# Sleepwalking/libllsm2

Hardware: AMD Instinct MI355X
Metric: frames/sec (layer0 analyze+synth, 44.1 kHz, 5 ms hop) (higher is better)
Workload: dtype f32; 1 GPU; 1024 synthetic 1 s utterances per GPU, F0 120 Hz fixed, 44.1 kHz, 5 ms hop, layer0 analyze+synth, default options, f0_refine=0; utterances_per_gpu=1024, frames_per_utterance=200, parallelism=dp1

## Files before the change

### libllsm2_amd/csrc/engine.cpp

```cpp
#include <hip/hip_runtime.h>
#include <sched.h>

#include <algorithm>
#include <atomic>
#include <cctype>
#include <cmath>
#include <cstdio>
#include <cstring>
#include <map>
#include <mutex>
#include <string>
#include <vector>

#include "cheby.h"
#include "engine.h"
#include "kernels.h"
#include "llsm_gpu.h"
#include "plan.h"
#include "batch.h"

namespace lp = llsm_plan;

namespace {
struct HostConventions { int hann_periodic = 0, mavg_half = 3, filtfilt_pad = 15, interp1u_excl = 0, kalman_init = 0, lobe_1e6 = 133979, lf_rd_clamp = 0; } g_hconv;
// ... 1136 lines not shown
      int C = (int)((Ftot + NF_UNIT_DIV - 1) / NF_UNIT_DIV);
      C = std::max(4, (C + 1) & ~1);
      if(const char* e = std::getenv("LLSM_GPU_NOISE_UNIT")) C = std::max(2, std::atoi(e) & ~1);
      std::vector<int4> units;
      for(int u = 0; u < b -> lay.n_utt; u ++) {
        const int nf = b -> nfrm[u], nu = (nf + C - 1) / C;
        const int sz = nu > 0 ? (((nf + nu - 1) / nu) + 1) & ~1 : 2;
        for(int i0 = 0; i0 < nf; i0 += sz) units.push_back(make_int4(u, i0, std::min(i0 + sz, nf), 0));
      }
      b -> n_nf_units = (int)units.size();
      const double hop = (double)thop * fs;
      b -> nf_halo = (int)std::floor((b -> nfft_filt + 1) / std::max(hop, 1.0));
      if(upload_vec(b -> nf_units, units)) return -1;
    }
    std::vector<float> wf = make_hann(b -> nwin_filt);
    double s = 0; for(float v : wf) s += (double)v * v;
    b -> inv_wsqr = (float)(1.0 / s);
    if(upload_vec(b -> win_filt, wf)) return -1;
    b -> syn_fs = fs; b -> njobs_syn = 0;
  }
  if(so -> use_l1 && llsm_l1_prefetch_rows(b, so)) return -1;
  const size_t tplsz = (size_t)L.n_utt * nch * L.ntemplate_ext;
  if(b -> colored.alloc(tplsz) || b -> mid.alloc(tplsz) ||
     b -> iir_tmp.alloc((size_t)L.n_utt * nch * (L.ntemplate_ext + 32)) ||
     b -> env_cplx.alloc(F * nch * std::max(L.maxnhar_e, 1)) || b -> yexc.alloc(Y)) return -1;
  float* white = (float*)b -> arr[LLSM_GPU_WHITE];
  {
    const void* key[3] = {b -> colored.p, b -> mid.p, b -> iir_tmp.p};
    if(b -> njobs_syn == 0 || std::memcmp(key, b -> key_syn, sizeof(key))) {
      if(build_jobs(b, 1, fs, nullptr, white)) return -1;
      std::memcpy(b -> key_syn, key, sizeof(key));
    }
  }
  BatchDev d = batch_dev(b, fs);
  LaunchCtx* P = & c -> lc;
  float* ysin = (float*)b -> arr[LLSM_GPU_YSIN];
  if(! use_injected_white) RUN(launch_white(P, d, white, L.ntemplate_ext, b -> d_ny.p, seed));
  RUN(launch_filtfilt(P, b -> jobs_syn.p, b -> njobs_syn, b -> sections.p));
  RUN(launch_env_params(P, d, b -> env_cplx.p));
  RUN(launch_excite_env(P, d, b -> colored.p, L.ntemplate_ext, b -> env_hits.p, b -> env_cplx.p,
    b -> nwin_env, b -> win_env.p, b -> nch_active, b -> d_y_off.p, b -> d_ny.p, b -> max_ny, fs,
    b -> yexc.p));
  float* ynoise = (float*)b -> arr[LLSM_GPU_YNOISE];
  static const bool fused_ok = [] { const char* e = std::getenv("LLSM_GPU_NOISE_OLA"); return !(e && e[0] == '0'); }();
  int fused = -2;
  if(fused_ok)
    fused = launch_noise_filter_ola(P, d, b -> nf_units.p, b -> n_nf_units, b -> nf_halo, b -> yexc.p,
      b -> d_y_off.p, b -> d_ny.p, b -> fnyq, fs, b -> nwin_filt, b -> win_filt.p, hann_sym(b -> nwin_filt), b -> inv_wsqr,
      ilog2(b -> nfft_filt), ynoise);
  if(fused != 0 && fused != -2) {
    llsm_set_error(std::string("launch_noise_filter_ola failed: ") + hipGetErrorString((hipError_t)fused));
    return -1;
  }
  float* yout = (float*)b -> arr[LLSM_GPU_Y];
  if(so -> use_l1) {
    if(fused == -2) {
      if(b -> nframes.alloc(F * b -> nfft_filt) || b -> live.alloc(F)) return -1;
      if(b -> nfft_filt > LLSM_LDS_FFT_MAX &&
         llsm_engine_big_fft(c, b -> nfft_filt, (size_t)llsm_big_fft_grid((size_t)b -> nfft_filt + b -> nfft_filt / 2 + 1) * (size_t)(b -> nfft_filt + b -> nfft_filt / 2 + 1))) return -1;
      HIP_OK(hipMemsetAsync(ysin, 0, Y * sizeof(float), c -> stream));
      RUN(launch_noise_filter(P, d, b -> yexc.p, b -> d_y_off.p, b -> d_ny.p, b -> fnyq, fs,
        b -> nwin_filt, b -> win_filt.p, b -> inv_wsqr, b -> nfft_filt, ilog2(b -> nfft_filt),
        c -> tw, c -> tw_nmax, b -> nframes.p, b -> live.p, 0));
      RUN(launch_ola_noise_mix(P, d, b -> nframes.p, b -> live.p, b -> nfft_filt,
        b -> d_y_off.p, b -> d_ny.p, b -> max_ny, fs, ysin, ynoise, yout));
    }
    return llsm_l1_synthesize_harmonics(b, so, ynoise, ysin, yout);
  }
  RUN(launch_synth_ola(P, d, b -> sin_units.p, b -> n_sin_units, b -> sin_halo, b -> nwin_sin, b -> win_sin.p,
    std::min(L.maxnhar, 2048), b -> d_y_off.p, b -> d_ny.p, fused == 0 ? ynoise : nullptr, ysin, 1,
    fused == 0 ? yout : nullptr));
  if(fused == -2) {
// ... 88 lines not shown
```

### libllsm2_amd/csrc/kernels.h

```cpp
#ifndef LLSM_AMD_KERNELS_H
#define LLSM_AMD_KERNELS_H

#include <hip/hip_runtime.h>
#include <stddef.h>
#include "cheby.h"
#include "packed.h"

struct FiltSectionD {
  double b[5];
  double a[5];
  double zi[4];
  double M[6][16];
  double H[IIR_SEG][4];
};

#ifndef KAL_CHUNK
#define KAL_CHUNK 8
#endif
struct FiltJob {
  const float* src;
  float* dst;
  float* mid;
  float* tmp;
  int n;
// ... 66 lines not shown
int launch_psd_frames(LaunchCtx* P, const BatchDev& d, const float* xres, int nwin,
  const float* win, float inv_wpow, int N, int logN, const float2* tw, int tw_nmax,
  float* psd_log);
int launch_kalman(LaunchCtx* P, const BatchDev& d, const float* env, const float* psd_log,
  float* ck, int nspec);
int launch_white(LaunchCtx* P, const BatchDev& d, float* white, int ntemplate_ext,
  const int* out_len, unsigned long long seed);
int launch_env_frames(LaunchCtx* P, const BatchDev& d, float fs_syn, int nwin,
  const float* win, float* envf);
#define LLSM_EXC_HITS 3
int launch_env_params(LaunchCtx* P, const BatchDev& d, float2* cplx);
int launch_pack_frames(LaunchCtx* P, const BatchDev& d, const LlsmPackedLayout& L, float* out, float* const* dst_tab);
int launch_unpack_frames(LaunchCtx* P, const BatchDev& d, const LlsmPackedLayout& L, const float* in, const float* const* src_tab);
int launch_scatter_outputs(LaunchCtx* P, int n_utt, int max_ny, const float* y, const float* ysin, const float* ynoise,
  const int* y_off, const int* ny, float* const* tab);
int launch_env_plan(LaunchCtx* P, int max_ny, int max_nfrm, int nwin_env, float thop, float fs, int2* hits, int* over);
int launch_excite_env(LaunchCtx* P, const BatchDev& d, const float* colored, int ntemplate_ext,
  const int2* hits, const float2* cplx, int nwin_env, const float* win, int nch_active,
  const int* out_off, const int* out_len, int max_len, float fs_syn, float* yexc);
int launch_noise_filter(LaunchCtx* P, const BatchDev& d, const float* yexc,
  const int* out_off, const int* out_len, float fnyq_conf, float fs_syn, int nwin,
  const float* win, float inv_wsqr, int N, int logN, const float2* tw, int tw_nmax,
  float* nframes_out, int* live, int rt);
int launch_noise_filter_ola(LaunchCtx* P, const BatchDev& d, const int4* units, int nunits, int halo,
  const float* yexc, const int* out_off, const int* out_len, float fnyq_conf, float fs_syn, int nwin,
  const float* win, int wsym, float inv_wsqr, int logN, float* ynoise);
int launch_ola_noise_mix(LaunchCtx* P, const BatchDev& d, const float* nframes_in,
  const int* live, int N, const int* out_off, const int* out_len,
  int max_len, float fs_syn, const float* ysin, float* ynoise, float* y);

int launch_utt_fftsize(LaunchCtx* P, const BatchDev& d, int nmax, int* nfft_u);
int launch_harm_pp(LaunchCtx* P, const BatchDev& d, const float* sig, size_t sig_stride, int nsig,
  const int* nfft_u, int maxnhar, float norm_base, const float2* tw, int tw_nmax, int lds_n,
  int* nhar_out, float* ampl, float* phse);
int launch_rt_template(LaunchCtx* P, const float* colored, int ntemplate_ext, int nch, int nch_active,
  int ntemplate, int S, float* tpl);
int launch_rt_rings(LaunchCtx* P, int S, float* mod, float* sinr, float* noiser, int cap, int nch,
  int mod_curr, int sin_curr, int noise_curr, int nhop, int nwin, const float* envf,
  const float* frames_sin, const float* f0, const int* has_nm, const int* nhar);
int launch_rt_rings_excite(LaunchCtx* P, int S, float* mod, float* sinr, float* noiser, int cap, int nch,
  int mod_curr, int sin_curr, int noise_curr, int nhop, int nwin, const float* envf, const float* frames_sin,
  const float* f0, const int* has_nm, const int* nhar, const float* tpl, float* excr, int ntemplate, int exc_curr,
  int exc_cycle, float* exc_frame);
int launch_rt_excite(LaunchCtx* P, int S, const float* mod, const float* tpl, float* excr, int cap,
  int nch, int ntemplate, int mod_curr, int exc_curr, int exc_cycle, int curr_nhop, int nx,
  int nwin_frame, float* exc_frame);
int launch_rt_mix(LaunchCtx* P, int S, float* noiser, const float* sinr, int cap, int noise_curr,
  int sin_curr, int sin_pos, int nfft, const float* nframes_in, const int* live, int next_nhop,
  int out_stride, float* out);
// ... 88 lines not shown
```

### libllsm2_amd/csrc/kernels.hip

```cpp
#include <hip/hip_runtime.h>
#include <stdint.h>
#include <climits>
#include <algorithm>
#include <cstdlib>
#include <cstring>
#include <map>
#include <mutex>
#include <utility>

#include "kernels.h"
#include "plan.h"

namespace lp = llsm_plan;

#pragma clang fp contract(fast)

#include "dev_common.h"
#include "synth_frame.h"
#include "launch.h"
#if defined(LLSM_KBENCH_EXPERIMENTS)
#include "../../tools/kbench_experiments.h"
#else
#if defined(IIR_FAKE_L2) || defined(IIR_GEN_EXPERIMENT) || defined(RT2_TIMING) || defined(HT_TABLE_EXPERIMENT) || defined(KAL_BREAK)
#error "timing-experiment switches need -DLLSM_KBENCH_EXPERIMENTS (tools/kbench.py); the product library is never built with them"
// ... 1983 lines not shown
__global__ __launch_bounds__(256) void k_env_params(
  const float* __restrict__ f0, const int* __restrict__ nhar_e,
  const float* __restrict__ eamp, const float* __restrict__ ephs, int nframes, int nch, int me,
  float2* __restrict__ cplx) {
  const size_t tid = (size_t)blockIdx.x * 256 + threadIdx.x;
  if(tid >= (size_t)nframes * nch * me) return;
  const int g = (int)(tid / ((size_t)nch * me)), k = (int)(tid % me);
  const int K = f0[g] > 0 ? min(nhar_e[g], me) : 0;
  float2 v = make_float2(0.0f, 0.0f);
  if(k < K) {
    float sn, co; sincosf(ephs[tid], & sn, & co);
    const float a = eamp[tid];
    v = make_float2(a * co, a * sn);
  }
  cplx[tid] = v;
}

#define EXC_HITS 3
#ifndef EXC_FAST
#define EXC_FAST 1
#endif
#define EXC_SLOTS 8
template <int NCH, int ME>
__global__ __launch_bounds__(256) void k_excite_env(
  const float* __restrict__ colored, int ntemplate_ext, const int2* __restrict__ hits,
  const float2* __restrict__ cplx, const float* __restrict__ edc, const float* __restrict__ f0,
  int nwin_env, const float* __restrict__ win, int nch, int me, int nch_active,
  const int* __restrict__ frm_off, const int* __restrict__ nfrm,
  const int* __restrict__ out_off, const int* __restrict__ out_len, float thop, float fs,
  float* __restrict__ yexc) {
  __shared__ float2 s_cp[EXC_SLOTS][NCH * ME];
  __shared__ float s_off[EXC_SLOTS][NCH];
  __shared__ float s_turn[EXC_SLOTS];
  const int u = blockIdx.y;
  const int b0 = blockIdx.x * 256, idx = b0 + threadIdx.x;
  const int ny = out_len[u];
  if(b0 >= ny) return;
  const int nf = nfrm[u], fo = frm_off[u];
  const float hop = lp::fmul(thop, fs);
  const int imin = max(0, (int)((float)b0 / hop) - 1);
  for(int t = threadIdx.x; t < EXC_SLOTS * NCH * ME; t += 256) {
    const int sl = t / (NCH * ME), r = t % (NCH * ME), c = r / ME, k = r % ME;
    const int i = imin + sl;
    float2 v = make_float2(0.0f, 0.0f);
    if(i < nf && c < nch && k < me) v = cplx[((size_t)(fo + i) * nch + c) * me + k];
    s_cp[sl][r] = v;
// ... 1 lines not shown
  if(threadIdx.x < EXC_SLOTS * NCH) {
    const int sl = threadIdx.x / NCH, c = threadIdx.x % NCH, i = imin + sl;
    s_off[sl][c] = (i < nf && c < nch) ? edc[(size_t)(fo + i) * nch + c] : 0.0f;
  }
  if(threadIdx.x < EXC_SLOTS) {
    const int i = imin + threadIdx.x;
    s_turn[threadIdx.x] = i < nf ? f0[fo + i] / fs : 0.0f;
  }
  __syncthreads();
  if(idx >= ny) return;
  const int ntemplate = min(20000, ny);
  int b; float r;
  const int a = lp::stretch_index(idx, ntemplate, ny, 128, & b, & r);
  const int half = nwin_env / 2;
  float e[NCH];
#pragma unroll
  for(int c = 0; c < NCH; c ++) e[c] = 0.0f;
#pragma unroll
  for(int hh = 0; hh < EXC_HITS; hh ++) {
    const int2 hit = hits[(size_t)idx * EXC_HITS + hh];
    if(hit.x < 0 || hit.x >= nf) continue;
    const int sl = hit.x - imin, j = hit.y;
    const float w = win[j];
    if(sl >= 0 && sl < EXC_SLOTS) {
      const float tn = s_turn[sl];
      float z1r = 1.0f, z1i = 0.0f;
#if EXC_FAST
      if(tn > 0) { const float ph = tn * (float)(j - half); z1r = __builtin_amdgcn_cosf(ph); z1i = __builtin_amdgcn_sinf(ph); }
#else
      if(tn > 0) cs_turns((double)tn * (double)(j - half), & z1r, & z1i);
#endif
      float zr[ME], zi[ME];
      zr[0] = z1r; zi[0] = z1i;
#pragma unroll
      for(int k = 1; k < ME; k ++) {
        zr[k] = zr[k - 1] * z1r - zi[k - 1] * z1i; zi[k] = zr[k - 1] * z1i + zi[k - 1] * z1r;
      }
#pragma unroll
      for(int c = 0; c < NCH; c ++) {
        float y = 0.0f;
#pragma unroll
        for(int k = 0; k < ME; k ++) {
          const float2 av = s_cp[sl][c * ME + k];
          y += av.x * zr[k] - av.y * zi[k];
        }
        e[c] += fmaxf(y + s_off[sl][c], 1e-8f) * w;
      }
    } else {
      const int g = fo + hit.x;
      const float f = f0[g];
      float z1r = 1.0f, z1i = 0.0f;
      if(f > 0) cs_turns((double)(f / fs) * (double)(j - half), & z1r, & z1i);
      for(int c = 0; c < nch; c ++) {
        float y = 0.0f, zr = z1r, zi = z1i;
        for(int k = 0; k < me; k ++) {
          const float2 av = cplx[((size_t)g * nch + c) * me + k];
          y += av.x * zr - av.y * zi;
          const float nr = zr * z1r - zi * z1i, ni = zr * z1i + zi * z1r;
          zr = nr; zi = ni;
        }
        const float val = fmaxf(y + edc[(size_t)g * nch + c], 1e-8f) * w;
#pragma unroll
        for(int cc = 0; cc < NCH; cc ++) if(cc == c) e[cc] += val;
      }
    }
  }
  const float xf = b >= 0 ? __frsqrt_rn(2.0f * r * (r - 1.0f) + 1.0f) : 1.0f;
  float acc = 0;
#pragma unroll
  for(int c = 0; c < NCH; c ++) {
    if(c < nch_active) {
      const float* tpl = colored + ((size_t)u * nch + c) * ntemplate_ext;
      float v = tpl[a];
      if(b >= 0) {
        v *= 1.0f - r;
        v += tpl[b] * r;
        v *= xf;
      }
#if EXC_FAST
      v *= __builtin_amdgcn_sqrtf(e[c]);
#else
      v *= sqrtf(e[c]);
#endif
      acc += v;
    }
  }
  yexc[(size_t)out_off[u] + idx] = acc;
}


#ifndef EXC4_WPE
#define EXC4_WPE 4
#endif
#define EXC4_SLOTS 16
template <int NCH, int ME>
__global__ __launch_bounds__(256, EXC4_WPE) void k_excite_env4(
  const float* __restrict__ colored, int ntemplate_ext, const int2* __restrict__ hits,
  const float2* __restrict__ cplx, const float* __restrict__ edc, const float* __restrict__ f0,
  int nwin_env, const float* __restrict__ win, int nch, int me, int nch_active,
  const int* __restrict__ frm_off, const int* __restrict__ nfrm,
  const int* __restrict__ out_off, const int* __restrict__ out_len, float thop, float fs,
  float* __restrict__ yexc) {
  __shared__ __attribute__((aligned(16))) float2 s_cp[EXC4_SLOTS][NCH * ME];
  __shared__ float s_off[EXC4_SLOTS][NCH];
  __shared__ float s_turn[EXC4_SLOTS];
  __shared__ float2 s_w[EXC4_SLOTS];
  const int u = blockIdx.y;
  const int ny = out_len[u];
  const int nt = min(20000, ny);
  const bool tiled = ny > nt;
// ... 515 lines not shown
      const int lo = max(0, k - mavg_h), hi = min(nspec - 1, k + mavg_h);
      const float inv = 1.0f / (float)(hi - lo + 1);
      ea *= inv; eb *= inv;
    }
    const float pos = (float)k * cpos;
    int q = (int)pos;
    float ta, tb;
    if(q >= npsd - 1) { const float2 t = Tdb[npsd - 1]; ta = t.x; tb = t.y; }
    else {
      const float rr = pos - (float)q;
      const float2 t0 = Tdb[q], t1 = Tdb[q + 1];
      ta = t0.x + (t1.x - t0.x) * rr; tb = t0.y + (t1.y - t0.y) * rr;
    }
    const float ha = __expf(ta * (2.3025851f / 20.0f)) * __frsqrt_rn(fmaf(ea, esc, 1e-8f));
    const float hb = __expf(tb * (2.3025851f / 20.0f)) * __frsqrt_rn(fmaf(eb, esc, 1e-8f));
    float ar = xr[m] * ha, ai = xi[m] * ha, br = mr[m] * hb, bi = mi[m] * hb;
    if(m == 0 && lane == 0) { ai = 0.0f; bi = 0.0f; }
    if(m == H - 1) { nyq_r = __shfl(ar, WAVE - 1, WAVE); nyq_i = __shfl(br, WAVE - 1, WAVE); }
    xr[m] = ar - bi; xi[m] = ai + br;
    mr[m] = ar + bi; mi[m] = br - ai;
  }
}

template <int LOGN, bool ALIAS, int TQ>
__global__ __launch_bounds__(WAVE, (LOGN >= 11 ? 1 : (ALIAS ? NF_OLA_WPE : NF_WPE))) void k_noise_filter_ola(
  const int4* __restrict__ units, int nunits, int halo,
  const float* __restrict__ yexc, const int* __restrict__ out_off, const int* __restrict__ out_len,
  const int* __restrict__ frm_off, const int* __restrict__ nfrm,
  const float* __restrict__ psd, const float* __restrict__ psdres,
  const int* __restrict__ has_psdres, int npsd, float fnyq_conf,
  float thop, float fs, int nwin, const float* __restrict__ win, int wsym, float inv_wsqr,
  float* __restrict__ ynoise) {
  constexpr int N = 1 << LOGN, P = N / WAVE, H = P / 2, nspec = N / 2 + 1;
  const int lane = threadIdx.x;
  float2* lds = (float2*)g_lds;
  float2* Pw = lds;
  float2* Tdb = ALIAS ? lds + (nspec + 6) : lds + wf_lds_elems<LOGN>();
  float* ring = ALIAS ? (float*)(lds + wf_lds_elems<LOGN>()) : (float*)(Tdb + npsd);
  WfTw<LOGN> tw; wf_init(tw, lane);
  const int nfade = 16;
  const float fn_syn = fs / 2.0f;
  const float invN = 1.0f / (float)N;
  const int shift = N / 2 - nwin / 2;
  float wv[ALIAS ? 1 : P];
  float* Wh = ring + N;
  const int whalf = wsym / 2;
  if constexpr (ALIAS) { for(int j = lane; j <= whalf; j += WAVE) Wh[j] = j < nwin ? win[j] : 0.0f; }
#pragma unroll
  for(int m = 0; m < P; m ++) {
    if constexpr (! ALIAS) wv[m] = ld_guard(win, lane + WAVE * m - shift, nwin, true);
    ring[lane + WAVE * m] = 0.0f;
  }
  const int4 unit = units[xcd_frame(blockIdx.x, gridDim.x)];
  const int u = unit.x, i0 = unit.y, i1 = unit.z;
  const int nf = nfrm[u], fo = frm_off[u], ny = out_len[u];
  const size_t yo = (size_t)out_off[u];
  const float* xs = yexc + yo;
  float* yn = ynoise + yo;
  const int own_lo = i0 == 0 ? 0 : min(max(lp::center(i0, thop, fs) - N / 2, 0), ny);
  const int own_hi = i1 >= nf ? ny : min(max(lp::center(i1, thop, fs) - N / 2, 0), ny);
  const int j0 = max(0, i0 - halo) & ~1;
  int flushed = lp::center(j0, thop, fs) - N / 2;
  auto advance = [&](int target) {
    for(int s = flushed + lane; s < target; s += WAVE) {
      const float v = ring[s & (N - 1)];
      ring[s & (N - 1)] = 0.0f;
      if(s >= own_lo && s < own_hi) yn[s] = v;
    }
    flushed = max(flushed, target);
  };
  const float cpos = fn_syn / ((float)(nspec - 1) * fnyq_conf) * (float)(npsd - 1);
  const int mavg_h = g_conv.mavg_half;
  const float esc = 44100.0f / fs;
  float sxr[P], sxi[P];
  float sp0[TQ], sp1[TQ], sr0[TQ], sr1[TQ];
  int hr_stg[2] = {0, 0};
  auto stage = [&](int jn, const int (&hrn)[2]) {
    const bool v0 = jn < i1, v1 = jn + 1 < i1;
    const int c0 = lp::center(jn, thop, fs), c1 = lp::center(jn + 1, thop, fs);
    const int b0 = c0 - nwin / 2, b1 = c1 - nwin / 2;
    const int lo0 = max(b0, 0), lo1 = max(b1, 0);
    const buf_t r0 = buf_range(xs, lo0, v0 ? min(b0 + nwin, ny) : lo0);
    const buf_t r1 = buf_range(xs, lo1, v1 ? min(b1 + nwin, ny) : lo1);
    int o0 = (lane - shift + b0 - lo0) * 4, o1 = (lane - shift + b1 - lo1) * 4;
    asm volatile("" : "+v"(o0), "+v"(o1));
#pragma unroll
    for(int m = 0; m < P; m ++) {
#if NF_ABL & 1
      sxr[m] = (float)(o0 + m + jn) * 1e-3f; sxi[m] = (float)(o1 + m - jn) * 1e-3f; (void)r0; (void)r1;
#else
      sxr[m] = ld_range_b(r0, o0 + 4 * WAVE * m);
      sxi[m] = ld_range_b(r1, o1 + 4 * WAVE * m);
#endif
    }
    if constexpr (ALIAS) {
      const size_t g0 = (size_t)(fo + jn) * npsd, g1 = (size_t)(fo + (v1 ? jn + 1 : jn)) * npsd;
      const int np = v0 ? npsd : 0;
      const buf_t p0 = buf_range(psd + g0, 0, np), p1 = buf_range(psd + g1, 0, np);
      const buf_t q0 = buf_range(psdres + g0, 0, hrn[0] ? np : 0), q1 = buf_range(psdres + g1, 0, hrn[1] ? np : 0);
#pragma unroll
      for(int i = 0; i < TQ; i ++) {
        const int q = lane + WAVE * i;
        sp0[i] = ld_range(p0, q); sp1[i] = ld_range(p1, q);
        sr0[i] = ld_range(q0, q); sr1[i] = ld_range(q1, q);
      }
    }
    hr_stg[0] = hrn[0]; hr_stg[1] = hrn[1];
  };
  int hr_nxt[2];
#pragma unroll
  for(int e = 0; e < 2; e ++) hr_nxt[e] = has_psdres[fo + min(j0 + e, nf - 1)];
  stage(j0, hr_nxt);
  for(int j = j0; j < i1; j += 2) {
    const bool valid1 = j + 1 < i1;
    const int gg[2] = {fo + j, fo + (valid1 ? j + 1 : j)};
    const int cen[2] = {lp::center(j, thop, fs), lp::center(j + 1, thop, fs)};
    const int hr[2] = {hr_stg[0], hr_stg[1]};
    float xr[P], xi[P];
#pragma unroll
    for(int m = 0; m < P; m ++) { xr[m] = sxr[m]; xi[m] = sxi[m]; }
    float pk0 = -3.0e38f, pk1 = -3.0e38f;
    float tq0[TQ], tq1[TQ];
    {
      if constexpr (ALIAS) {
#pragma unroll
        for(int i = 0; i < TQ; i ++) {
          const int q = lane + WAVE * i;
          float t0 = -3.0e38f, t1 = -3.0e38f;
          if(q < npsd) {
            t0 = sp0[i]; t1 = sp1[i];
            pk0 = fmaxf(pk0, t0); pk1 = fmaxf(pk1, t1);
            if(hr[0]) t0 += sr0[i] - 1.6286014f;
            if(hr[1]) t1 += sr1[i] - 1.6286014f;
          }
          tq0[i] = t0; tq1[i] = t1;
        }
      } else {
        const size_t r0 = (size_t)gg[0] * npsd, r1 = (size_t)gg[1] * npsd;
        for(int q = lane; q < npsd; q += WAVE) {
          float t0 = psd[r0 + q], t1 = psd[r1 + q];
          pk0 = fmaxf(pk0, t0); pk1 = fmaxf(pk1, t1);
          if(hr[0]) t0 += psdres[r0 + q] - 1.6286014f;
          if(hr[1]) t1 += psdres[r1 + q] - 1.6286014f;
          Tdb[q] = make_float2(t0, t1);
        }
      }
    }
#pragma unroll
    for(int e = 0; e < 2; e ++) hr_nxt[e] = has_psdres[fo + min(j + 2 + e, nf - 1)];
    pk0 = wave_max(pk0); pk1 = wave_max(pk1);
    const bool alive[2] = {!(pk0 < -100.0f), valid1 && !(pk1 < -100.0f)};
    if(! alive[0] && ! alive[1]) { stage(j + 2, hr_nxt); continue; }
    {
      int js = lane - shift;
      asm volatile("" : "+v"(js));
#pragma unroll
      for(int m = 0; m < P; m ++) {
        float w;
        if constexpr (ALIAS) { const int j = js + WAVE * m; w = Wh[max(0, min(j, wsym - j))]; }
        else w = wv[m];
        xr[m] *= alive[0] ? w : 0.0f; xi[m] *= alive[1] ? w : 0.0f;
      }
    }
#if !(NF_ABL & 2)
    wave_fft<LOGN>(xr, xi, tw, lds, lane);
#endif
    float mr[H + 1], mi[H + 1];
    wave_mirror_lo<P>(xr, mr, lane);
    wave_mirror_lo<P>(xi, mi, lane);
    if(lane < 3) { Pw[lane] = make_float2(0.0f, 0.0f); Pw[nspec + 3 + lane] = make_float2(0.0f, 0.0f); }
    if constexpr (ALIAS) {
#pragma unroll
      for(int i = 0; i < TQ; i ++) if(lane + WAVE * i < npsd) Tdb[lane + WAVE * i] = make_float2(tq0[i], tq1[i]);
    }
#pragma unroll
// ... 24 lines not shown
    asm volatile("" : "+v"(lo_));
#pragma unroll
    for(int e = 0; e < 2; e ++) {
      if(! alive[e]) continue;
      const int st = cen[e] - N / 2;
#if NF_ABL & 16
      { float sacc = 0; for(int m = 0; m < P; m ++) sacc += (e == 0 ? xr[m] : xi[m]); if(sacc == 1.2345f) yn[lane] = sacc; continue; }
#endif
      advance(st);
      float acc[P];
#pragma unroll
      for(int m = 0; m < P; m ++) acc[m] = ring[(st + lo_ + WAVE * m) & (N - 1)];
#pragma unroll
      for(int m = 0; m < P; m ++) {
        const int t = lo_ + WAVE * m;
        float v = (e == 0 ? xr[m] : xi[m]) * invN;
        if(m == 0 && t < nfade) v *= (float)t / (float)nfade;
        if(m == P - 1 && t >= N - nfade) v *= 1.0f - (float)(N - 1 - t) / (float)nfade;
        acc[m] += v;
      }
#pragma unroll
      for(int m = 0; m < P; m ++) ring[(st + lo_ + WAVE * m) & (N - 1)] = acc[m];
    }
  }
  advance(own_hi);
}

__global__ __launch_bounds__(256) void k_ola_noise_mix(
  const float* __restrict__ nframes_in, const int* __restrict__ live, int N,
  const int* __restrict__ frm_off, const int* __restrict__ nfrm,
  const int* __restrict__ out_off, const int* __restrict__ out_len,
  float thop, float fs, const float* __restrict__ ysin,
  float* __restrict__ ynoise, float* __restrict__ y) {
  const int u = blockIdx.y;
  const int idx = blockIdx.x * 256 + threadIdx.x;
  if(idx >= out_len[u]) return;
  const int nf = nfrm[u], fo = frm_off[u];
  const float hop = lp::fmul(thop, fs);
  const size_t o = (size_t)out_off[u] + idx;
  const int ilo = max(0, (int)((float)(idx - N / 2) / hop) - 1);
  const int ihi = min(nf - 1, (int)((float)(idx + N / 2) / hop) + 1);
  float acc = 0;
  for(int i0 = ilo; i0 <= ihi; i0 += 8) {
    int lv[8]; float gv[8];
#pragma unroll
    for(int q = 0; q < 8; q ++) lv[q] = live[fo + min(i0 + q, nf - 1)];
// ... 906 lines not shown
  const int np = rt ? (d.nframes + 1) / 2 : npairs_of(d);
  if(N > LLSM_LDS_FFT_MAX) {
    const int grid = std::min(fft_grid(np), llsm_big_fft_grid((size_t)N + N / 2 + 1));
    if(! P -> tw_big || N > P -> tw_big_nmax || P -> big_scratch_elems < (size_t)grid * (N + N / 2 + 1)) return -1;
    LAUNCH("k_noise_filter", k_noise_filter, dim3(grid), dim3(WAVE), 64,
      yexc, out_off, out_len, d.frm_utt, d.frm_off, d.nframes, d.psd, d.psdres, d.has_psdres,
      d.npsd, fnyq_conf, d.thop, fs_syn, nwin, win, inv_wsqr, N, logN, P -> tw_big, P -> tw_big_nmax,
      nframes_out, live, rt, rt ? nullptr : d.pairs, np, P -> big_scratch);
    return 0;
  }
  size_t lds = (size_t)(N + N / 2 + N / 2 + 1) * sizeof(float2) + 16 * sizeof(float);
  lds = (lds + 15) / 16 * 16;
  if(lds > 64 * 1024 &&
     hipFuncSetAttribute((const void*)k_noise_filter, hipFuncAttributeMaxDynamicSharedMemorySize, (int)lds) != hipSuccess) return -1;
  LAUNCH("k_noise_filter", k_noise_filter, dim3(fft_grid(np)), dim3(WAVE), lds,
    yexc, out_off, out_len, d.frm_utt, d.frm_off, d.nframes, d.psd, d.psdres, d.has_psdres,
    d.npsd, fnyq_conf, d.thop, fs_syn, nwin, win, inv_wsqr, N, logN, tw, tw_nmax,
    nframes_out, live, rt, rt ? nullptr : d.pairs, np, (float2*)nullptr);
  return 0;
}

int launch_noise_filter_ola(LaunchCtx* P, const BatchDev& d, const int4* units, int nunits, int halo,
  const float* yexc, const int* out_off, const int* out_len, float fnyq_conf, float fs_syn, int nwin,
  const float* win, int wsym, float inv_wsqr, int logN, float* ynoise) {
  if(nunits == 0) return 0;
#define NFO_ARGS units, nunits, halo, yexc, out_off, out_len, d.frm_off, d.nfrm, d.psd, d.psdres, d.has_psdres, d.npsd, fnyq_conf, \
      d.thop, fs_syn, nwin, win, wsym, inv_wsqr, ynoise
#define WF_CASE(LN) \
  if(logN == LN) { \
     \
    if(wsym > 0 && d.npsd <= NF_TQ * WAVE && (1 << (LN - 1)) + 7 + d.npsd <= wf_lds_elems<LN>()) { \
      if(d.npsd <= 2 * WAVE) { \
        LAUNCH("k_noise_filter_ola", (k_noise_filter_ola<LN, true, 2>), dim3(nunits), dim3(WAVE), \
          sizeof(float2) * wf_lds_elems<LN>() + (sizeof(float) << LN) + sizeof(float) * (wsym / 2 + 1), NFO_ARGS); \
      } else { \
        LAUNCH("k_noise_filter_ola", (k_noise_filter_ola<LN, true, NF_TQ>), dim3(nunits), dim3(WAVE), \
          sizeof(float2) * wf_lds_elems<LN>() + (sizeof(float) << LN) + sizeof(float) * (wsym / 2 + 1), NFO_ARGS); \
      } \
    } else { \
      LAUNCH("k_noise_filter_ola", (k_noise_filter_ola<LN, false, 1>), dim3(nunits), dim3(WAVE), \
        sizeof(float2) * (wf_lds_elems<LN>() + d.npsd) + (sizeof(float) << LN), NFO_ARGS); \
    } \
    return 0; \
  }
  WF_CASE(8) WF_CASE(9) WF_CASE(10) WF_CASE(11)
#undef WF_CASE
#undef NFO_ARGS
  return -2;
}

int launch_ola_noise_mix(LaunchCtx* P, const BatchDev& d, const float* nframes_in,
  const int* live, int N, const int* out_off, const int* out_len,
  int max_len, float fs_syn, const float* ysin, float* ynoise, float* y) {
  if(d.n_utt == 0 || max_len == 0) return 0;
  LAUNCH("k_ola_noise_mix", k_ola_noise_mix, dim3((max_len + 255) / 256, d.n_utt), dim3(256), 0,
    nframes_in, live, N, d.frm_off, d.nfrm, out_off, out_len, d.thop, fs_syn, ysin, ynoise, y);
  return 0;
}

int launch_rt_template(LaunchCtx* P, const float* colored, int ntemplate_ext, int nch, int nch_active,
  int ntemplate, int S, float* tpl) {
  LAUNCH("k_rt_template", k_rt_template, dim3((ntemplate + 255) / 256, nch, S), dim3(256), 0,
    colored, ntemplate_ext, nch, nch_active, ntemplate, tpl);
  return 0;
}
int launch_rt_rings(LaunchCtx* P, int S, float* mod, float* sinr, float* noiser, int cap, int nch,
  int mod_curr, int sin_curr, int noise_curr, int nhop, int nwin, const float* envf,
  const float* frames_sin, const float* f0, const int* has_nm, const int* nhar) {
  LAUNCH("k_rt_rings", k_rt_rings, dim3(S), dim3(256), 0, mod, sinr, noiser, cap, nch, mod_curr,
    sin_curr, noise_curr, nhop, nwin, envf, frames_sin, f0, has_nm, nhar);
  return 0;
// ... 176 lines not shown
```

Measured before the change: 34.89 million frames/s.

## Fuse excitation envelope synthesis into the noise filter OLA kernel

Computes the envelope-modulated noise excitation on the fly inside k_noise_filter_ola, writing it to an LDS ring buffer instead of materialising yexc in global memory. This removes the env_params and excite_env launches and the global write and re-read of the excitation signal. The excite helpers are factored into shared device functions so both paths use the same math. In exchange the fused kernel uses more LDS and registers, and it falls back to the old path under several shape conditions.

```diff
diff --git a/libllsm2_amd/csrc/engine.cpp b/libllsm2_amd/csrc/engine.cpp
--- a/libllsm2_amd/csrc/engine.cpp
+++ b/libllsm2_amd/csrc/engine.cpp
@@ -1182,8 +1182,7 @@
   if(so -> use_l1 && llsm_l1_prefetch_rows(b, so)) return -1;
   const size_t tplsz = (size_t)L.n_utt * nch * L.ntemplate_ext;
   if(b -> colored.alloc(tplsz) || b -> mid.alloc(tplsz) ||
-     b -> iir_tmp.alloc((size_t)L.n_utt * nch * (L.ntemplate_ext + 32)) ||
-     b -> env_cplx.alloc(F * nch * std::max(L.maxnhar_e, 1)) || b -> yexc.alloc(Y)) return -1;
+     b -> iir_tmp.alloc((size_t)L.n_utt * nch * (L.ntemplate_ext + 32))) return -1;
   float* white = (float*)b -> arr[LLSM_GPU_WHITE];
   {
     const void* key[3] = {b -> colored.p, b -> mid.p, b -> iir_tmp.p};
@@ -1197,17 +1196,30 @@
   float* ysin = (float*)b -> arr[LLSM_GPU_YSIN];
   if(! use_injected_white) RUN(launch_white(P, d, white, L.ntemplate_ext, b -> d_ny.p, seed));
   RUN(launch_filtfilt(P, b -> jobs_syn.p, b -> njobs_syn, b -> sections.p));
-  RUN(launch_env_params(P, d, b -> env_cplx.p));
-  RUN(launch_excite_env(P, d, b -> colored.p, L.ntemplate_ext, b -> env_hits.p, b -> env_cplx.p,
-    b -> nwin_env, b -> win_env.p, b -> nch_active, b -> d_y_off.p, b -> d_ny.p, b -> max_ny, fs,
-    b -> yexc.p));
   float* ynoise = (float*)b -> arr[LLSM_GPU_YNOISE];
   static const bool fused_ok = [] { const char* e = std::getenv("LLSM_GPU_NOISE_OLA"); return !(e && e[0] == '0'); }();
-  int fused = -2;
-  if(fused_ok)
-    fused = launch_noise_filter_ola(P, d, b -> nf_units.p, b -> n_nf_units, b -> nf_halo, b -> yexc.p,
+  const char* ef = std::getenv("LLSM_GPU_NOISE_FUSED");
+  const char* e4 = std::getenv("LLSM_GPU_EXCITE4");
+  const bool fuse_exc = fused_ok && !(ef && ef[0] == '0') && !(e4 && e4[0] == '1');
+  int fused = -3;
+  if(fuse_exc) {
+    const NfExc x{b -> colored.p, L.ntemplate_ext, b -> env_hits.p, b -> win_env.p, b -> nwin_env, hann_sym(b -> nwin_env), b -> nch_active};
+    fused = launch_noise_filter_ola(P, d, b -> nf_units.p, b -> n_nf_units, b -> nf_halo, nullptr,
       b -> d_y_off.p, b -> d_ny.p, b -> fnyq, fs, b -> nwin_filt, b -> win_filt.p, hann_sym(b -> nwin_filt), b -> inv_wsqr,
-      ilog2(b -> nfft_filt), ynoise);
+      ilog2(b -> nfft_filt), ynoise, & x);
+  }
+  if(fused == -3) {
+    if(b -> env_cplx.alloc(F * nch * std::max(L.maxnhar_e, 1)) || b -> yexc.alloc(Y)) return -1;
+    RUN(launch_env_params(P, d, b -> env_cplx.p));
+    RUN(launch_excite_env(P, d, b -> colored.p, L.ntemplate_ext, b -> env_hits.p, b -> env_cplx.p,
+      b -> nwin_env, b -> win_env.p, b -> nch_active, b -> d_y_off.p, b -> d_ny.p, b -> max_ny, fs,
+      b -> yexc.p));
+    fused = -2;
+    if(fused_ok)
+      fused = launch_noise_filter_ola(P, d, b -> nf_units.p, b -> n_nf_units, b -> nf_halo, b -> yexc.p,
+        b -> d_y_off.p, b -> d_ny.p, b -> fnyq, fs, b -> nwin_filt, b -> win_filt.p, hann_sym(b -> nwin_filt), b -> inv_wsqr,
+        ilog2(b -> nfft_filt), ynoise, nullptr);
+  }
   if(fused != 0 && fused != -2) {
     llsm_set_error(std::string("launch_noise_filter_ola failed: ") + hipGetErrorString((hipError_t)fused));
     return -1;
diff --git a/libllsm2_amd/csrc/kernels.h b/libllsm2_amd/csrc/kernels.h
--- a/libllsm2_amd/csrc/kernels.h
+++ b/libllsm2_amd/csrc/kernels.h
@@ -112,9 +112,15 @@
   const int* out_off, const int* out_len, float fnyq_conf, float fs_syn, int nwin,
   const float* win, float inv_wsqr, int N, int logN, const float2* tw, int tw_nmax,
   float* nframes_out, int* live, int rt);
+struct NfExc {
+  const float* colored; int ntemplate_ext;
+  const int2* hits;
+  const float* win_env; int nwin_env, wsym_env;
+  int nch_active;
+};
 int launch_noise_filter_ola(LaunchCtx* P, const BatchDev& d, const int4* units, int nunits, int halo,
   const float* yexc, const int* out_off, const int* out_len, float fnyq_conf, float fs_syn, int nwin,
-  const float* win, int wsym, float inv_wsqr, int logN, float* ynoise);
+  const float* win, int wsym, float inv_wsqr, int logN, float* ynoise, const NfExc* x);
 int launch_ola_noise_mix(LaunchCtx* P, const BatchDev& d, const float* nframes_in,
   const int* live, int N, const int* out_off, const int* out_len,
   int max_len, float fs_syn, const float* ysin, float* ynoise, float* y);
diff --git a/libllsm2_amd/csrc/kernels.hip b/libllsm2_amd/csrc/kernels.hip
--- a/libllsm2_amd/csrc/kernels.hip
+++ b/libllsm2_amd/csrc/kernels.hip
@@ -2029,6 +2029,56 @@
 #endif
 #define EXC_SLOTS 8
 template <int NCH, int ME>
+DEV void exc_env_hit(float (&e)[NCH], const float2* cp, const float* off, float tn, int jrel, float w) {
+#pragma clang fp contract(off)
+  float z1r = 1.0f, z1i = 0.0f;
+#if EXC_FAST
+  if(tn > 0) { const float ph = tn * (float)jrel; z1r = __builtin_amdgcn_cosf(ph); z1i = __builtin_amdgcn_sinf(ph); }
+#else
+  if(tn > 0) cs_turns((double)tn * (double)jrel, & z1r, & z1i);
+#endif
+  float zr[ME], zi[ME];
+  zr[0] = z1r; zi[0] = z1i;
+#pragma unroll
+  for(int k = 1; k < ME; k ++) {
+    zr[k] = zr[k - 1] * z1r - zi[k - 1] * z1i; zi[k] = zr[k - 1] * z1i + zi[k - 1] * z1r;
+  }
+#pragma unroll
+  for(int c = 0; c < NCH; c ++) {
+    float y = 0.0f;
+#pragma unroll
+    for(int k = 0; k < ME; k ++) {
+      const float2 av = cp[c * ME + k];
+      y += av.x * zr[k] - av.y * zi[k];
+    }
+    e[c] += fmaxf(y + off[c], 1e-8f) * w;
+  }
+}
+template <int NCH>
+DEV float exc_mix(const float (&e)[NCH], const float (&va)[NCH], const float (&vb)[NCH], float rf, int nch_active) {
+#pragma clang fp contract(off)
+  const float xf = rf >= 0 ? __frsqrt_rn(2.0f * rf * (rf - 1.0f) + 1.0f) : 1.0f;
+  float acc = 0;
+#pragma unroll
+  for(int c = 0; c < NCH; c ++) {
+    if(c < nch_active) {
+      float v = va[c];
+      if(rf >= 0) {
+        v *= 1.0f - rf;
+        v += vb[c] * rf;
+        v *= xf;
+      }
+#if EXC_FAST
+      v *= __builtin_amdgcn_sqrtf(e[c]);
+#else
+      v *= sqrtf(e[c]);
+#endif
+      acc += v;
+    }
+  }
+  return acc;
+}
+template <int NCH, int ME>
 __global__ __launch_bounds__(256) void k_excite_env(
   const float* __restrict__ colored, int ntemplate_ext, const int2* __restrict__ hits,
   const float2* __restrict__ cplx, const float* __restrict__ edc, const float* __restrict__ f0,
@@ -2076,31 +2126,8 @@
     if(hit.x < 0 || hit.x >= nf) continue;
     const int sl = hit.x - imin, j = hit.y;
     const float w = win[j];
-    if(sl >= 0 && sl < EXC_SLOTS) {
-      const float tn = s_turn[sl];
-      float z1r = 1.0f, z1i = 0.0f;
-#if EXC_FAST
-      if(tn > 0) { const float ph = tn * (float)(j - half); z1r = __builtin_amdgcn_cosf(ph); z1i = __builtin_amdgcn_sinf(ph); }
-#else
-      if(tn > 0) cs_turns((double)tn * (double)(j - half), & z1r, & z1i);
-#endif
-      float zr[ME], zi[ME];
-      zr[0] = z1r; zi[0] = z1i;
-#pragma unroll
-      for(int k = 1; k < ME; k ++) {
-        zr[k] = zr[k - 1] * z1r - zi[k - 1] * z1i; zi[k] = zr[k - 1] * z1i + zi[k - 1] * z1r;
-      }
-#pragma unroll
-      for(int c = 0; c < NCH; c ++) {
-        float y = 0.0f;
-#pragma unroll
-        for(int k = 0; k < ME; k ++) {
-          const float2 av = s_cp[sl][c * ME + k];
-          y += av.x * zr[k] - av.y * zi[k];
-        }
-        e[c] += fmaxf(y + s_off[sl][c], 1e-8f) * w;
-      }
-    } else {
+    if(sl >= 0 && sl < EXC_SLOTS) exc_env_hit<NCH, ME>(e, s_cp[sl], s_off[sl], s_turn[sl], j - half, w);
+    else {
       const int g = fo + hit.x;
       const float f = f0[g];
       float z1r = 1.0f, z1i = 0.0f;
@@ -2119,27 +2146,17 @@
       }
     }
   }
-  const float xf = b >= 0 ? __frsqrt_rn(2.0f * r * (r - 1.0f) + 1.0f) : 1.0f;
-  float acc = 0;
+  float va[NCH], vb[NCH];
 #pragma unroll
   for(int c = 0; c < NCH; c ++) {
+    va[c] = 0.0f; vb[c] = 0.0f;
     if(c < nch_active) {
       const float* tpl = colored + ((size_t)u * nch + c) * ntemplate_ext;
-      float v = tpl[a];
-      if(b >= 0) {
-        v *= 1.0f - r;
-        v += tpl[b] * r;
-        v *= xf;
-      }
-#if EXC_FAST
-      v *= __builtin_amdgcn_sqrtf(e[c]);
-#else
-      v *= sqrtf(e[c]);
-#endif
-      acc += v;
-    }
-  }
-  yexc[(size_t)out_off[u] + idx] = acc;
+      va[c] = tpl[a];
+      if(b >= 0) vb[c] = tpl[b];
+    }
+  }
+  yexc[(size_t)out_off[u] + idx] = exc_mix<NCH>(e, va, vb, b >= 0 ? r : -1.0f, nch_active);
 }
 
 
@@ -2701,7 +2718,17 @@
   }
 }
 
-template <int LOGN, bool ALIAS, int TQ>
+#define NFX_QS 7
+#define NFX_SLOTS 12
+struct NfExcDev {
+  const float* colored; int ntemplate_ext; const int2* hits;
+  const float* f0; const int* nhar_e; const float* eamp; const float* ephs; const float* edc;
+  const float* win_env; int nwin_env, wsym_env, nch, me, nch_active, R;
+};
+template <int XME> constexpr int nfx_stage_floats() { return 2 * NFX_SLOTS * 4 * XME + NFX_SLOTS * 4 + 2 * NFX_SLOTS; }
+template <int LOGN> constexpr int nfx_xmax() { return nfx_stage_floats<8>() <= 2 * wf_lds_elems<LOGN>() ? 8 : 4; }
+
+template <int LOGN, bool ALIAS, int TQ, int XME>
 __global__ __launch_bounds__(WAVE, (LOGN >= 11 ? 1 : (ALIAS ? NF_OLA_WPE : NF_WPE))) void k_noise_filter_ola(
   const int4* __restrict__ units, int nunits, int halo,
   const float* __restrict__ yexc, const int* __restrict__ out_off, const int* __restrict__ out_len,
@@ -2709,8 +2736,10 @@
   const float* __restrict__ psd, const float* __restrict__ psdres,
   const int* __restrict__ has_psdres, int npsd, float fnyq_conf,
   float thop, float fs, int nwin, const float* __restrict__ win, int wsym, float inv_wsqr,
-  float* __restrict__ ynoise) {
+  float* __restrict__ ynoise, NfExcDev xa) {
   constexpr int N = 1 << LOGN, P = N / WAVE, H = P / 2, nspec = N / 2 + 1;
+  constexpr bool FX = XME > 0;
+  static_assert(! FX || (ALIAS && nfx_stage_floats<XME>() <= 2 * wf_lds_elems<LOGN>()), "fused excitation: ALIAS form, staging inside the exchange buffer");
   const int lane = threadIdx.x;
   float2* lds = (float2*)g_lds;
   float2* Pw = lds;
@@ -2734,7 +2763,7 @@
   const int u = unit.x, i0 = unit.y, i1 = unit.z;
   const int nf = nfrm[u], fo = frm_off[u], ny = out_len[u];
   const size_t yo = (size_t)out_off[u];
-  const float* xs = yexc + yo;
+  const float* xs = FX ? nullptr : yexc + yo;
   float* yn = ynoise + yo;
   const int own_lo = i0 == 0 ? 0 : min(max(lp::center(i0, thop, fs) - N / 2, 0), ny);
   const int own_hi = i1 >= nf ? ny : min(max(lp::center(i1, thop, fs) - N / 2, 0), ny);
@@ -2751,7 +2780,106 @@
   const float cpos = fn_syn / ((float)(nspec - 1) * fnyq_conf) * (float)(npsd - 1);
   const int mavg_h = g_conv.mavg_half;
   const float esc = 44100.0f / fs;
-  float sxr[P], sxi[P];
+  float* X = Wh + whalf + 1;
+  float* We = X + xa.R;
+  constexpr int XM = FX ? XME : 1, XQ = FX ? NFX_QS : 1, XNP = FX ? (NFX_SLOTS * 4 * XM + WAVE - 1) / WAVE : 1;
+  if constexpr (FX) { for(int j = lane; j <= xa.wsym_env / 2; j += WAVE) We[j] = j < xa.nwin_env ? xa.win_env[j] : 0.0f; }
+  const float hop = lp::fmul(thop, fs);
+  const int ntemplate = min(20000, ny), half_e = xa.nwin_env / 2;
+  int xp = max(lp::center(j0, thop, fs) - nwin / 2, 0);
+  int x_tgt = xp;
+  int x_lo = 0, x_hi = 0, x_imin = 0;
+  float xva[XQ][4], xrf[XQ];
+  float xpa[XNP], xpp[XNP], xf0 = 0.0f, xedc = 0.0f;
+  int xnh = 0;
+  auto xload = [&](int lo, int hi) __attribute__((always_inline)) {
+    x_lo = lo; x_hi = min(hi, lo + XQ * WAVE);
+    x_imin = max(0, (int)((float)lo / hop) - 1);
+#pragma unroll
+    for(int q = 0; q < XQ; q ++) {
+      const int p = max(0, min(lo + lane + WAVE * q, ny - 1));
+      int bb; float r;
+      const int a = lp::stretch_index(p, ntemplate, ny, 128, & bb, & r);
+      xrf[q] = bb >= 0 ? r : -1.0f;
+#pragma unroll
+      for(int c = 0; c < 4; c ++) xva[q][c] = c < xa.nch_active ? xa.colored[((size_t)u * xa.nch + c) * xa.ntemplate_ext + a] : 0.0f;
+    }
+#pragma unroll
+    for(int t = 0; t < XNP; t ++) {
+      const int e = lane + WAVE * t, sl = e / (4 * XM), r = e % (4 * XM), c = r / XM, k = r % XM, i = x_imin + sl;
+      const bool ok = sl < NFX_SLOTS && i < nf && c < xa.nch && k < xa.me;
+      const size_t o = ok ? ((size_t)(fo + i) * xa.nch + c) * xa.me + k : 0;
+      xpa[t] = ok ? xa.eamp[o] : 0.0f; xpp[t] = ok ? xa.ephs[o] : 0.0f;
+    }
+    {
+      const int i = x_imin + lane, ie = x_imin + lane / 4, c = lane % 4;
+      xf0 = lane < NFX_SLOTS && i < nf ? xa.f0[fo + i] : 0.0f;
+      xnh = lane < NFX_SLOTS && i < nf ? xa.nhar_e[fo + i] : 0;
+      xedc = lane < NFX_SLOTS * 4 && ie < nf && c < xa.nch ? xa.edc[(size_t)(fo + ie) * xa.nch + c] : 0.0f;
+    }
+  };
+  auto xfinish = [&]() __attribute__((always_inline)) {
+    float2* cpS = lds;
+    float* offS = (float*)(cpS + NFX_SLOTS * 4 * XM);
+    float* turnS = offS + NFX_SLOTS * 4;
+    int* kS = (int*)(turnS + NFX_SLOTS);
+    int2 xh[XQ][EXC_HITS];
+#pragma unroll
+    for(int q = 0; q < XQ; q ++) {
+      const int p = max(0, min(x_lo + lane + WAVE * q, ny - 1));
+#pragma unroll
+      for(int hh = 0; hh < EXC_HITS; hh ++) xh[q][hh] = xa.hits[(size_t)p * EXC_HITS + hh];
+    }
+    __syncthreads();
+    if(lane < NFX_SLOTS) { turnS[lane] = x_imin + lane < nf ? xf0 / fs : 0.0f; kS[lane] = xf0 > 0 ? min(xnh, xa.me) : 0; }
+    if(lane < NFX_SLOTS * 4) offS[lane] = xedc;
+    __syncthreads();
+#pragma unroll
+    for(int t = 0; t < XNP; t ++) {
+      const int e = lane + WAVE * t;
+      if(e < NFX_SLOTS * 4 * XM) {
+        float2 v = make_float2(0.0f, 0.0f);
+        if(e % XM < kS[e / (4 * XM)]) {
+          float sn, co; sincosf(xpp[t], & sn, & co);
+          const float a = xpa[t];
+          v = make_float2(a * co, a * sn);
+        }
+        cpS[e] = v;
+      }
+    }
+    __syncthreads();
+#pragma unroll
+    for(int q = 0; q < XQ; q ++) {
+      float e[4] = {0.0f, 0.0f, 0.0f, 0.0f};
+#pragma unroll
+      for(int hh = 0; hh < EXC_HITS; hh ++) {
+        const int2 hit = xh[q][hh];
+        if(hit.x < 0 || hit.x >= nf) continue;
+        const int sl = max(0, min(hit.x - x_imin, NFX_SLOTS - 1)), j = hit.y;
+        const float w = We[min(j, xa.wsym_env - j)];
+        exc_env_hit<4, XM>(e, cpS + sl * 4 * XM, offS + sl * 4, turnS[sl], j - half_e, w);
+      }
+      const int p = x_lo + lane + WAVE * q;
+      float vb[4] = {0.0f, 0.0f, 0.0f, 0.0f};
+      if(xrf[q] >= 0) {
+        int bb; float r;
+        lp::stretch_index(max(0, min(p, ny - 1)), ntemplate, ny, 128, & bb, & r);
+#pragma unroll
+        for(int c = 0; c < 4; c ++) if(c < xa.nch_active) vb[c] = xa.colored[((size_t)u * xa.nch + c) * xa.ntemplate_ext + bb];
+      }
+      const float v = exc_mix<4>(e, xva[q], vb, xrf[q], xa.nch_active);
+      if(p < x_hi) X[p & (xa.R - 1)] = v;
+    }
+    __syncthreads();
+    xp = max(xp, x_hi);
+  };
+  auto produce = [&]() __attribute__((always_inline)) {
+    if constexpr (FX) {
+      xfinish();
+      while(xp < x_tgt) { xload(xp, x_tgt); xfinish(); }
+    }
+  };
+  float sxr[FX ? 1 : P], sxi[FX ? 1 : P];
   float sp0[TQ], sp1[TQ], sr0[TQ], sr1[TQ];
   int hr_stg[2] = {0, 0};
   auto stage = [&](int jn, const int (&hrn)[2]) {
@@ -2759,6 +2887,10 @@
     const int c0 = lp::center(jn, thop, fs), c1 = lp::center(jn + 1, thop, fs);
     const int b0 = c0 - nwin / 2, b1 = c1 - nwin / 2;
     const int lo0 = max(b0, 0), lo1 = max(b1, 0);
+    if constexpr (FX) {
+      x_tgt = max(xp, v1 ? min(b1 + nwin, ny) : (v0 ? min(b0 + nwin, ny) : 0));
+      xload(xp, x_tgt);
+    } else {
     const buf_t r0 = buf_range(xs, lo0, v0 ? min(b0 + nwin, ny) : lo0);
     const buf_t r1 = buf_range(xs, lo1, v1 ? min(b1 + nwin, ny) : lo1);
     int o0 = (lane - shift + b0 - lo0) * 4, o1 = (lane - shift + b1 - lo1) * 4;
@@ -2772,6 +2904,7 @@
       sxi[m] = ld_range_b(r1, o1 + 4 * WAVE * m);
 #endif
     }
+    }
     if constexpr (ALIAS) {
       const size_t g0 = (size_t)(fo + jn) * npsd, g1 = (size_t)(fo + (v1 ? jn + 1 : jn)) * npsd;
       const int np = v0 ? npsd : 0;
@@ -2790,14 +2923,29 @@
 #pragma unroll
   for(int e = 0; e < 2; e ++) hr_nxt[e] = has_psdres[fo + min(j0 + e, nf - 1)];
   stage(j0, hr_nxt);
+  produce();
   for(int j = j0; j < i1; j += 2) {
     const bool valid1 = j + 1 < i1;
     const int gg[2] = {fo + j, fo + (valid1 ? j + 1 : j)};
     const int cen[2] = {lp::center(j, thop, fs), lp::center(j + 1, thop, fs)};
     const int hr[2] = {hr_stg[0], hr_stg[1]};
     float xr[P], xi[P];
-#pragma unroll
-    for(int m = 0; m < P; m ++) { xr[m] = sxr[m]; xi[m] = sxi[m]; }
+    if constexpr (FX) {
+      const int b0 = cen[0] - nwin / 2, b1 = cen[1] - nwin / 2;
+      const int lo0 = max(b0, 0), hi0 = min(b0 + nwin, ny), lo1 = max(b1, 0), hi1 = valid1 ? min(b1 + nwin, ny) : lo1;
+      int s0 = b0 + lane - shift;
+      asm volatile("" : "+v"(s0));
+      const int d1 = b1 - b0;
+#pragma unroll
+      for(int m = 0; m < P; m ++) {
+        const int s = s0 + WAVE * m, t = s + d1;
+        xr[m] = (s >= lo0 && s < hi0) ? X[s & (xa.R - 1)] : 0.0f;
+        xi[m] = (t >= lo1 && t < hi1) ? X[t & (xa.R - 1)] : 0.0f;
+      }
+    } else {
+#pragma unroll
+      for(int m = 0; m < P; m ++) { xr[m] = sxr[m]; xi[m] = sxi[m]; }
+    }
     float pk0 = -3.0e38f, pk1 = -3.0e38f;
     float tq0[TQ], tq1[TQ];
     {
@@ -2829,7 +2977,7 @@
     for(int e = 0; e < 2; e ++) hr_nxt[e] = has_psdres[fo + min(j + 2 + e, nf - 1)];
     pk0 = wave_max(pk0); pk1 = wave_max(pk1);
     const bool alive[2] = {!(pk0 < -100.0f), valid1 && !(pk1 < -100.0f)};
-    if(! alive[0] && ! alive[1]) { stage(j + 2, hr_nxt); continue; }
+    if(! alive[0] && ! alive[1]) { stage(j + 2, hr_nxt); produce(); continue; }
     {
       int js = lane - shift;
       asm volatile("" : "+v"(js));
@@ -2900,6 +3048,7 @@
 #pragma unroll
       for(int m = 0; m < P; m ++) ring[(st + lo_ + WAVE * m) & (N - 1)] = acc[m];
     }
+    produce();
   }
   advance(own_hi);
 }
@@ -3852,31 +4001,68 @@
 
 int launch_noise_filter_ola(LaunchCtx* P, const BatchDev& d, const int4* units, int nunits, int halo,
   const float* yexc, const int* out_off, const int* out_len, float fnyq_conf, float fs_syn, int nwin,
-  const float* win, int wsym, float inv_wsqr, int logN, float* ynoise) {
+  const float* win, int wsym, float inv_wsqr, int logN, float* ynoise, const NfExc* x) {
+  NfExcDev xd{};
+  if(x) {
+    const float hop = lp::fmul(d.thop, fs_syn);
+    const int span = nwin + (int)std::ceil(hop) + 1;
+    int R = 1; while(R < span) R *= 2;
+    if(logN > 10 || d.nchannel > 4 || d.maxnhar_e > 8 || x -> wsym_env <= 0 || ! (wsym > 0) ||
+       hop * (NFX_SLOTS - 5) < (float)(NFX_QS * WAVE) || nwin <= hop + 1) return -3;
+    xd = NfExcDev{x -> colored, x -> ntemplate_ext, x -> hits, d.f0, d.nhar_e, d.eenv_ampl, d.eenv_phse, d.edc,
+                  x -> win_env, x -> nwin_env, x -> wsym_env, d.nchannel, d.maxnhar_e, x -> nch_active, R};
+  }
   if(nunits == 0) return 0;
 #define NFO_ARGS units, nunits, halo, yexc, out_off, out_len, d.frm_off, d.nfrm, d.psd, d.psdres, d.has_psdres, d.npsd, fnyq_conf, \
-      d.thop, fs_syn, nwin, win, wsym, inv_wsqr, ynoise
+      d.thop, fs_syn, nwin, win, wsym, inv_wsqr, ynoise, xd
+#define NFO_ALIAS_LDS(LN) (sizeof(float2) * wf_lds_elems<LN>() + (sizeof(float) << LN) + sizeof(float) * (wsym / 2 + 1))
 #define WF_CASE(LN) \
   if(logN == LN) { \
+    constexpr int XMAX = nfx_xmax<LN>(); \
      \
-    if(wsym > 0 && d.npsd <= NF_TQ * WAVE && (1 << (LN - 1)) + 7 + d.npsd <= wf_lds_elems<LN>()) { \
+    const bool alias = wsym > 0 && d.npsd <= NF_TQ * WAVE && (1 << (LN - 1)) + 7 + d.npsd <= wf_lds_elems<LN>(); \
+    if(x) { \
+      const size_t lds = NFO_ALIAS_LDS(LN) + sizeof(float) * (xd.R + x -> wsym_env / 2 + 1); \
+      const int xme = d.maxnhar_e <= 4 ? 4 : 8; \
+      if(! alias || lds > 20 * 1024 || xme > XMAX) return -3; \
       if(d.npsd <= 2 * WAVE) { \
-        LAUNCH("k_noise_filter_ola", (k_noise_filter_ola<LN, true, 2>), dim3(nunits), dim3(WAVE), \
-          sizeof(float2) * wf_lds_elems<LN>() + (sizeof(float) << LN) + sizeof(float) * (wsym / 2 + 1), NFO_ARGS); \
+        if(xme == 4) LAUNCH("k_noise_filter_ola", (k_noise_filter_ola<LN, true, 2, 4>), dim3(nunits), dim3(WAVE), lds, NFO_ARGS); \
+        else LAUNCH("k_noise_filter_ola", (k_noise_filter_ola<LN, true, 2, (XMAX)>), dim3(nunits), dim3(WAVE), lds, NFO_ARGS); \
       } else { \
-        LAUNCH("k_noise_filter_ola", (k_noise_filter_ola<LN, true, NF_TQ>), dim3(nunits), dim3(WAVE), \
-          sizeof(float2) * wf_lds_elems<LN>() + (sizeof(float) << LN) + sizeof(float) * (wsym / 2 + 1), NFO_ARGS); \
+        if(xme == 4) LAUNCH("k_noise_filter_ola", (k_noise_filter_ola<LN, true, NF_TQ, 4>), dim3(nunits), dim3(WAVE), lds, NFO_ARGS); \
+        else LAUNCH("k_noise_filter_ola", (k_noise_filter_ola<LN, true, NF_TQ, (XMAX)>), dim3(nunits), dim3(WAVE), lds, NFO_ARGS); \
+      } \
+      return 0; \
+    } \
+    if(alias) { \
+      if(d.npsd <= 2 * WAVE) { \
+        LAUNCH("k_noise_filter_ola", (k_noise_filter_ola<LN, true, 2, 0>), dim3(nunits), dim3(WAVE), NFO_ALIAS_LDS(LN), NFO_ARGS); \
+      } else { \
+        LAUNCH("k_noise_filter_ola", (k_noise_filter_ola<LN, true, NF_TQ, 0>), dim3(nunits), dim3(WAVE), NFO_ALIAS_LDS(LN), NFO_ARGS); \
       } \
     } else { \
-      LAUNCH("k_noise_filter_ola", (k_noise_filter_ola<LN, false, 1>), dim3(nunits), dim3(WAVE), \
+      LAUNCH("k_noise_filter_ola", (k_noise_filter_ola<LN, false, 1, 0>), dim3(nunits), dim3(WAVE), \
         sizeof(float2) * (wf_lds_elems<LN>() + d.npsd) + (sizeof(float) << LN), NFO_ARGS); \
     } \
     return 0; \
   }
-  WF_CASE(8) WF_CASE(9) WF_CASE(10) WF_CASE(11)
+  WF_CASE(8) WF_CASE(9) WF_CASE(10)
 #undef WF_CASE
+#define WF_CASE(LN) \
+  if(logN == LN) { \
+    if(x) return -3; \
+    const bool alias = wsym > 0 && d.npsd <= NF_TQ * WAVE && (1 << (LN - 1)) + 7 + d.npsd <= wf_lds_elems<LN>(); \
+    if(alias && d.npsd <= 2 * WAVE) LAUNCH("k_noise_filter_ola", (k_noise_filter_ola<LN, true, 2, 0>), dim3(nunits), dim3(WAVE), NFO_ALIAS_LDS(LN), NFO_ARGS); \
+    else if(alias) LAUNCH("k_noise_filter_ola", (k_noise_filter_ola<LN, true, NF_TQ, 0>), dim3(nunits), dim3(WAVE), NFO_ALIAS_LDS(LN), NFO_ARGS); \
+    else LAUNCH("k_noise_filter_ola", (k_noise_filter_ola<LN, false, 1, 0>), dim3(nunits), dim3(WAVE), \
+        sizeof(float2) * (wf_lds_elems<LN>() + d.npsd) + (sizeof(float) << LN), NFO_ARGS); \
+    return 0; \
+  }
+  WF_CASE(11)
+#undef WF_CASE
+#undef NFO_ALIAS_LDS
 #undef NFO_ARGS
-  return -2;
+  return x ? -3 : -2;
 }
 
 int launch_ola_noise_mix(LaunchCtx* P, const BatchDev& d, const float* nframes_in,
```

Result: no change. 34.43 million frames/s, median of 6 (-1.3%).
